# leodd/Lifted-Hybrid-Variational-Inference

Hardware: AMD Instinct MI355X
Metric: lbp_sweeps_per_sec_10M_edge_hybrid_mrf (higher is better)
Workload: dtype f64

## Files before the change

include/lhvi.h:

```cpp
#ifndef LHVI_H
#define LHVI_H

#include <stddef.h>
#include <stdint.h>

#ifdef __cplusplus
extern "C" {
#endif

#define LHVI_ABI_VERSION 30
#define LHVI_MAX_ARITY 6

#define LHVI_OK 0
#define LHVI_E_ARG (-1)
#define LHVI_E_LAUNCH (-2)
#define LHVI_E_UNSUPPORTED (-3)
#define LHVI_E_NODEVICE (-4)
#define LHVI_E_NOT_PD (-5)

#define LHVI_POT_GENERIC 0
#define LHVI_POT_TABLE 1
#define LHVI_POT_GAUSSIAN 2
#define LHVI_POT_QUADRATIC 3
#define LHVI_POT_HYBRID_QUADRATIC 4
#define LHVI_POT_LINEAR_GAUSSIAN 5
#define LHVI_POT_X2 6
#define LHVI_POT_XY 7
#define LHVI_POT_MLN 8
#define LHVI_POT_MLN_HARD 9
#define LHVI_POT_IMAGE_NODE 10
#define LHVI_POT_IMAGE_EDGE 11

typedef struct lhvi_graph {
    int32_t V, F, E, nnz;
    const int32_t* fac_ptr;
    const int32_t* edge_var;
    const int32_t* edge_fac;
    const int32_t* edge_canon;
    const int32_t* var_ptr;
    const int32_t* var_edge;
    const double* edge_count;
    const int32_t* fac_pot;
    const double* var_value;
    const int32_t* var_dom;
    const double* var_mult;
    const double* fac_mult;
    int32_t D;
    const int32_t* dom_cont;
    const double* dom_lo;
    const double* dom_hi;
    const int32_t* dom_ptr;
    const double* dom_val;
    const double* edge_value;
    const int32_t* slot_var;
    const int32_t* hub_vars;
    int32_t n_hubs;
} lhvi_graph_t;
#define LHVI_HUB_DEGREE 64

typedef struct lhvi_pots {
    int32_t P;
    const int32_t* kind;
    const int32_t* off;
// ... 8 lines not shown


int lhvi_gabp_init(const lhvi_graph_t* g, double* f2v, double* v2f, void* stream);
int lhvi_gabp_v2f(const lhvi_graph_t* g, const double* f2v, double* v2f, void* stream);
int lhvi_gabp_f2v(const lhvi_graph_t* g, const lhvi_pots_t* pots, const double* v2f, double* f2v, void* stream);
int lhvi_gabp_run(const lhvi_graph_t* g, const lhvi_pots_t* pots, double* f2v, double* v2f, int iterations, void* stream);
typedef struct lhvi_gabp_plan {
    const int32_t* pslot;
    const int32_t* info;
    const double* count;
    int32_t n_hub_rows;
    const int32_t* rec;
    const double* pot_words;
    const int32_t* seg;
    int32_t n_seg;
} lhvi_gabp_plan_t;
size_t lhvi_gabp_pull_workspace_bytes(const lhvi_graph_t* g);
int lhvi_gabp_pull(const lhvi_graph_t* g, const lhvi_pots_t* pots, const lhvi_gabp_plan_t* plan, const double* v_prev,
                   double* v_next, int first, void* stream);
int lhvi_gabp_run_pull(const lhvi_graph_t* g, const lhvi_pots_t* pots, const lhvi_gabp_plan_t* plan, double* f2v, double* v2f,
                       int iterations, void* ws, size_t ws_bytes, void* stream);

int lhvi_gabp_graph_create(const lhvi_graph_t* g, const lhvi_pots_t* pots, const lhvi_gabp_plan_t* plan, double* f2v, double* v2f,
                           double* mu_var, int iterations, void* ws, size_t ws_bytes, void** handle_out);
int lhvi_gabp_graph_launch(void* handle, void* stream);
int lhvi_gabp_graph_destroy(void* handle);

int lhvi_gabp_marginals(const lhvi_graph_t* g, const double* f2v, double* mu_var, void* stream);

size_t lhvi_log_likelihood_workspace_bytes(const lhvi_graph_t* g);
int lhvi_log_likelihood(const lhvi_graph_t* g, const lhvi_pots_t* pots, const double* x, double* out, void* ws, size_t ws_bytes,
                        void* stream);


#define LHVI_PBP_EP 1u
#define LHVI_PBP_EPBP_DISCRETE 2u
#define LHVI_PBP_SKIP_TERMS 16u
#define LHVI_PBP_LEAVE_ROOM 256u
#define LHVI_PBP_CQ 512u
#define LHVI_PBP_BOUNDARY_TOTALS 2048u
#define LHVI_PBP_NO_UNIQ 4096u
#define LHVI_PBP_V2F_RECORDS 8192u
#define LHVI_PBP_WIDE_PAIRS 16384u
#define LHVI_PBP_SHARE_CUS 32768u
#define LHVI_PBP_NO_GRID 128u
#define LHVI_PBP_FUSED_RECORDS16 131072u
#define LHVI_PBP_F2V_HEAVY 262144u
#define LHVI_PBP_F2V_SMALL 524288u
#define LHVI_PBP_F2V_PAIR 1048576u
#define LHVI_PBP_F2V_FAST 2097152u
#define LHVI_PBP_F2V_CQ 4194304u
#define LHVI_PBP_F2V_GENERIC 8388608u
#define LHVI_PBP_F2V_ALL (LHVI_PBP_F2V_HEAVY | LHVI_PBP_F2V_SMALL | LHVI_PBP_F2V_PAIR | LHVI_PBP_F2V_FAST | LHVI_PBP_F2V_CQ | LHVI_PBP_F2V_GENERIC)
#define LHVI_PBP_POW2_GROUPS 65536u

typedef struct lhvi_pbp {
    int32_t n;
    int32_t T;
    uint32_t flags;
    double var_threshold;
    double max_log_value;
    const double* particles;
    const double* old_particles;
    const int32_t* np;
    const uint8_t* uniq;
    const double* q;
    const int32_t* fast_edges;
    int32_t n_fast;
    const int32_t* generic_edges;
    int32_t n_generic;
    int32_t generic_pts_log2;
    const void* fast_desc;
    const void* heavy_desc;
    int32_t n_heavy;
    const void* light_desc;
    int32_t n_light;
    const int32_t* bslot;
    const int32_t* brow_ptr;
    const int64_t* brow_off;
    const int32_t* brow_peer;
    const double* recv;
    int32_t rank;
    const double* var_degree;
    int32_t var_lo, var_hi;
    uint32_t* f2v_ticket;
    const int32_t* prop_desc;
    int32_t n_prop_desc;
    const void* pair_desc;
    int32_t n_pair;
    const void* cq_desc;
    int32_t n_cq;
    const int32_t* v2f_wide;
    int32_t n_v2f_wide;
    const int32_t* v2f_narrow;
    int32_t n_v2f_narrow;
    const int32_t* v2f_hub;
    int32_t n_v2f_hub;
    const int32_t* v2f_mid16;
    int32_t n_v2f_mid16;
    const int32_t* v2f_mid32;
    int32_t n_v2f_mid32;
    const int32_t* prop_hub;
    int32_t n_prop_hub;
    double* prop_partial;
    const int32_t* resample_vars;
    int32_t n_resample_vars;
// ... 400 lines not shown
```

lifted-hybrid-variational-inference_amd/csrc/pbp.hip:

```cpp
#include "common.hpp"
#include "potential.hpp"
#include "fastmath.hpp"
#include "cq.hpp"
#include "gk21.hpp"

namespace lhvi {

__device__ __forceinline__ double wave_sum(double v) { return dpp_wave_reduce(v, SumOp()); }
__device__ __forceinline__ double wave_max(double v) { return dpp_wave_reduce(v, MaxOp()); }
__device__ __forceinline__ int wave_sum_i(int v) {
#pragma unroll
    for (int off = 32; off > 0; off >>= 1) v += __shfl_xor(v, off);
    return v;
}

constexpr double PAD_LOG_TERM = -6.0e5;

__host__ __device__ __forceinline__ int var_first(const lhvi_pbp_t& s) { return s.var_hi > s.var_lo ? s.var_lo : 0; }
__host__ __device__ __forceinline__ int var_limit(const lhvi_graph_t& g, const lhvi_pbp_t& s) { return s.var_hi > s.var_lo ? s.var_hi : g.V; }

__device__ __forceinline__ double norm_pdf_std(double x, double mu, double sig) {
    const double u = (x - mu) / sig;
    return exp(-u * u * 0.5) / (2.506628274631 * sig);
}
// ... 2697 lines not shown
#pragma unroll
        for (int off = PW; off < 64; off <<= 1) { fs += __shfl_xor(fs, off); fm += __shfl_xor(fm, off); }
    } else if (PW == 16 && SL == 1) { fs = (ps[0] + ps[1]) + (ps[2] + ps[3]); fm = (pm[0] + pm[1]) + (pm[2] + pm[3]); }
    else if (PW == 16) {
        const double s01 = (sub == 0 ? ps[0] : ps[1]), s23 = (sub == 0 ? ps[2] : ps[3]);
        const double m01 = (sub == 0 ? pm[0] : pm[1]), m23 = (sub == 0 ? pm[2] : pm[3]);
        fs = (s01 + __shfl_xor(s01, 16)) + (s23 + __shfl_xor(s23, 16));
        fm = (m01 + __shfl_xor(m01, 16)) + (m23 + __shfl_xor(m23, 16));
    } else { fs = ps[0] + ps[1]; fm = pm[0] + pm[1]; }
    fs = 1.0 / fs;
    const double mu_new = fs * fm, var_new = fs;
    if (on && j == 0) { q[2 * v] = mu_new; q[2 * v + 1] = var_new; }
    if constexpr (LATE_TABLE) {
        static_assert(LOG_TAB_N <= BLOCK, "one table entry per thread");
        if (threadIdx.x < LOG_TAB_N) { sh_log[threadIdx.x].inv_c = tab_inv; sh_log[threadIdx.x].log_c = tab_log; }
        __syncthreads();
    }
    const double mu_b = __shfl(mu_new, first_lane), sd_b = sqrt_pos(__shfl(var_new, first_lane));
    double x = 0.0;
    if (valid) {
        double zc, zs;
        philox_normal_pair(seed, gid ? (uint64_t)gid[v] : (uint64_t)v, (uint32_t)(W == 64 ? j & 31 : j), iteration, sh_log, zc, zs);
        if (W == 64 && (j & 32)) zc = zs;
        x = fmin(fmax(fma(sd_b, zc, mu_b), dlo), dhi) + 0.0;
        out[(int64_t)v * n + j] = x;
    }
    int u = valid;
    if constexpr (W == 64) {
        volatile uint8_t* owner = sh_owner + ((threadIdx.x >> 6) << FUSED64_HASH_BITS);
        const int xlo = __double2loint(x), xhi = __double2hiint(x);
        const uint32_t h = (((uint32_t)xlo * 0x9E3779B1u) ^ ((uint32_t)xhi * 0x85EBCA6Bu)) >> (32 - FUSED64_HASH_BITS);
        if (valid) owner[h] = (uint8_t)lane;
        LHVI_WAVE_SYNC();
        const bool suspect = valid && owner[h] != (uint8_t)lane;
        const uint64_t live = __ballot(valid);
        uint64_t todo = __ballot(suspect), dp = 0;
        while (todo) {
            const int k = __builtin_ctzll(todo);
            const int klo = __builtin_amdgcn_readlane(xlo, k), khi = __builtin_amdgcn_readlane(xhi, k);
            const uint64_t same = __ballot(xlo == klo && xhi == khi) & live;
            dp |= same & (same - 1);
            todo &= ~same;
        }
        u = valid && !((dp >> lane) & 1);
    } else {
        for (int k = 0; k + 1 < W; ++k) {
            const double xk = __shfl(x, first_lane + k);
            if (k < j && k < np && xk == x) u = 0;
        }
    }
    if (on && j < n) uniq[(int64_t)v * n + j] = (uint8_t)u;
}

}

#include "gmkl_dev.hpp"

namespace lhvi {

struct BeliefQ {
    const lhvi_graph_t& g; const lhvi_pots_t& pots; const lhvi_pbp_t& s; const double* __restrict__ v2f; const QueryRows& rows;
    int64_t i; int v; double logz; bool valid;

    template <class C> __device__ __forceinline__ void scan(const C&, const gmkl::Row&, gmkl::Scan& sc) const {
        sc.anyq = true;
        sc.bad = sc.bad || !valid;
    }
    __device__ __forceinline__ static int slots(const gmkl::Row&) { return 0; }
    template <class C> __device__ __forceinline__ void load_resident(const C&, const gmkl::Row&) const {}
    template <class C> __device__ __forceinline__ void eval(const C&, const gmkl::Row&, double x, double& m, double& sum) const {
        m = query_log_belief(g, pots, s, v2f, rows, i, v, x) - logz, sum = 1.0;
    }
};

__global__ void __launch_bounds__(WAVE, 2) pbp_kl_kernel(lhvi_graph_t g, lhvi_pots_t pots, lhvi_pbp_t s, const double* __restrict__ v2f,
                                                      QueryRows rows, const int32_t* __restrict__ row_var,
                                                      const double* __restrict__ logz, int32_t Kp, const double* __restrict__ wp,
                                                      const double* __restrict__ mup, const double* __restrict__ varp,
                                                      const double* __restrict__ a, const double* __restrict__ b, double epsabs,
                                                      double epsrel, double* __restrict__ kl, double* __restrict__ abserr,
                                                      int32_t* __restrict__ status, int32_t* __restrict__ neval) {
    __shared__ gmkl::Shared sh;
    const int64_t r = blockIdx.x;
    if (threadIdx.x == 0) {
        sh.in = gmkl::Row{Kp, 0, wp + r * Kp, mup + r * Kp, varp + r * Kp, nullptr, nullptr, nullptr, a[r], b[r], epsabs, epsrel};
        sh.kl = kl + r, sh.abserr = abserr ? abserr + r : nullptr;
        sh.status = status ? status + r : nullptr, sh.neval = neval ? neval + r : nullptr;
    }
    __syncthreads();
    gmkl::Row in = sh.in;
    in.Kp = Kp, in.Kq = 0;
    const int v = row_var[r];
    const double lz = logz[r];
    bool valid = v >= 0 && v < g.V && fabs(lz) <= DBL_MAX;
    if (valid) valid = is_hidden(g.var_value[v]) && g.dom_cont[g.var_dom[v]] != 0;
    const BeliefQ q{g, pots, s, v2f, rows, r, v, lz, valid};
    gmkl::DevCtx<BeliefQ> ctx(sh, (int)threadIdx.x, q);
    gmkl::kl_row(in, ctx, sh.kl, sh.abserr, sh.status, sh.neval);
}

static int validate_pbp(const lhvi_graph_t* g, const lhvi_pbp_t* s) {
    if (!g || !s) return LHVI_E_ARG;
    if (g->V < 0 || g->E < 0 || s->n <= 0 || s->T < 0) return LHVI_E_ARG;
    if (g->V > 0 && (!g->var_ptr || !g->var_edge || !g->var_value || !g->var_dom || !g->dom_cont || !g->dom_ptr ||
                     !s->particles || !s->np)) return LHVI_E_ARG;
    if (s->var_hi > s->var_lo ? (s->var_lo < 0 || s->var_hi > g->V) : (s->var_lo != 0 || s->var_hi != 0)) return LHVI_E_ARG;
// ... 384 lines not shown
                       row_var, xtol / 3.0, maxfun, xout, fout, nfev);
    return check_launch();
}

int lhvi_pbp_var_fused(const lhvi_graph_t* g, const lhvi_pbp_t* s, const double* f2v, double* v2f, double* eta, double* q,
                       const int64_t* var_gid, uint64_t seed, uint32_t iteration, double* particles_out, uint8_t* uniq_out,
                       const int32_t* desc, int32_t n16, int32_t n32_t32, int32_t n32_t64, void* stream) {
    if (int rc = validate_pbp(g, s)) return rc;
    if (!f2v || !v2f || !eta || !q || !particles_out || !uniq_out || !s->uniq || !s->q || !g->dom_lo || !g->dom_hi || !g->dom_val) return LHVI_E_ARG;
    if (n16 < 0 || n32_t32 < 0 || n32_t64 < 0 || s->n > 32 || s->bslot || s->var_hi > s->var_lo || particles_out == s->particles) return LHVI_E_ARG;
    if ((int64_t)n16 + n32_t32 + n32_t64 == 0) return LHVI_OK;
    if (!desc) return LHVI_E_ARG;
    hipStream_t st = as_stream(stream);
    const bool ep = (s->flags & LHVI_PBP_EP) != 0;
#define LHVI_FUSED(W, PW, list, cnt)                                                                                                  \
    if ((cnt) > 0) {                                                                                                                  \
        const dim3 grid(grid_for(((int64_t)(cnt) + WAVE / (W) - 1) / (WAVE / (W)) * WAVE));                                          \
        if (ep && r16) hipLaunchKernelGGL((pbp_var_fused_kernel<W, PW, true, true>), grid, dim3(BLOCK), 0, st, *g, *s, f2v, v2f, eta, q, var_gid, \
                                   seed, iteration, particles_out, uniq_out, list, cnt);                                             \
        else if (ep) hipLaunchKernelGGL((pbp_var_fused_kernel<W, PW, true, false>), grid, dim3(BLOCK), 0, st, *g, *s, f2v, v2f, eta, q, var_gid, \
                                   seed, iteration, particles_out, uniq_out, list, cnt);                                             \
        else if (r16) hipLaunchKernelGGL((pbp_var_fused_kernel<W, PW, false, true>), grid, dim3(BLOCK), 0, st, *g, *s, f2v, v2f, eta, q, var_gid,   \
                                seed, iteration, particles_out, uniq_out, list, cnt);                                                \
        else hipLaunchKernelGGL((pbp_var_fused_kernel<W, PW, false, false>), grid, dim3(BLOCK), 0, st, *g, *s, f2v, v2f, eta, q, var_gid,   \
                                seed, iteration, particles_out, uniq_out, list, cnt);                                                \
    }
    const bool r16 = (s->flags & LHVI_PBP_FUSED_RECORDS16) != 0;
    const int64_t rw = r16 ? 16 : 8;
    LHVI_FUSED(16, 16, desc, n16)
    LHVI_FUSED(32, 16, desc + rw * (int64_t)n16, n32_t32)
    LHVI_FUSED(32, 32, desc + rw * ((int64_t)n16 + n32_t32), n32_t64)
#undef LHVI_FUSED
    return check_launch();
}

int lhvi_pbp_var_fused64(const lhvi_graph_t* g, const lhvi_pbp_t* s, const double* f2v, double* v2f, double* eta, double* q,
                         const int64_t* var_gid, uint64_t seed, uint32_t iteration, double* particles_out, uint8_t* uniq_out,
                         const int32_t* desc, int32_t n64_t32, int32_t n64_t64, void* stream) {
    if (int rc = validate_pbp(g, s)) return rc;
    if (!f2v || !v2f || !eta || !q || !particles_out || !uniq_out || !s->uniq || !s->q || !g->dom_lo || !g->dom_hi || !g->dom_val) return LHVI_E_ARG;
    if (n64_t32 < 0 || n64_t64 < 0 || s->n <= 32 || s->n > 64 || s->bslot || s->var_hi > s->var_lo || particles_out == s->particles) return LHVI_E_ARG;
    if ((int64_t)n64_t32 + n64_t64 == 0) return LHVI_OK;
    if (!desc) return LHVI_E_ARG;
    hipStream_t st = as_stream(stream);
    const bool ep = (s->flags & LHVI_PBP_EP) != 0;
#define LHVI_FUSED64(PW, list, cnt)                                                                                                   \
    if ((cnt) > 0) {                                                                                                                  \
        const dim3 grid(grid_for((int64_t)(cnt) * WAVE));                                                                             \
        if (ep) hipLaunchKernelGGL((pbp_var_fused_kernel<64, PW, true, true>), grid, dim3(BLOCK), 0, st, *g, *s, f2v, v2f, eta, q, var_gid, \
                                   seed, iteration, particles_out, uniq_out, list, cnt);                                             \
        else hipLaunchKernelGGL((pbp_var_fused_kernel<64, PW, false, true>), grid, dim3(BLOCK), 0, st, *g, *s, f2v, v2f, eta, q, var_gid,   \
                                seed, iteration, particles_out, uniq_out, list, cnt);                                                \
    }
    LHVI_FUSED64(16, desc, n64_t32)
    LHVI_FUSED64(32, desc + 16 * (int64_t)n64_t32, n64_t64)
#undef LHVI_FUSED64
    return check_launch();
}

int lhvi_pbp_quad(const lhvi_graph_t* g, const lhvi_pots_t* pots, const lhvi_pbp_t* s, const double* v2f, int64_t nq,
                  const int32_t* row_var, const int64_t* qptr, const int32_t* qedge, const double* qmult, const double* lo,
                  const double* hi, double epsabs, double epsrel, double* z, double* abserr, int32_t* status, void* stream) {
    if (int rc = validate_pbp(g, s)) return rc;
    if (!pots || !v2f || nq < 0 || !(epsabs >= 0.0) || !(epsrel >= 0.0)) return LHVI_E_ARG;
    if (nq == 0) return LHVI_OK;
    if (!row_var || !lo || !hi || !z) return LHVI_E_ARG;
    if (qptr && (!qedge || !qmult)) return LHVI_E_ARG;
    QueryRows rows{row_var, qptr, qedge, qmult};
    hipLaunchKernelGGL(pbp_quad_kernel, dim3(grid_for(nq)), dim3(BLOCK), 0, as_stream(stream), *g, *pots, *s, v2f, nq, rows, row_var,
                       lo, hi, epsabs, epsrel, z, abserr, status);
    return check_launch();
}

int lhvi_pbp_kl(const lhvi_graph_t* g, const lhvi_pots_t* pots, const lhvi_pbp_t* s, const double* v2f, int64_t nq,
                const int32_t* row_var, const int64_t* qptr, const int32_t* qedge, const double* qmult, const double* logz,
                int32_t Kp, const double* wp, const double* mup, const double* varp, const double* a, const double* b,
                double epsabs, double epsrel, double* kl, double* abserr, int32_t* status, int32_t* neval, void* stream) {
    if (int rc = validate_pbp(g, s)) return rc;
    if (!pots || !v2f || nq < 1 || nq > 0x7fffffff || Kp < 1 || !(epsabs >= 0.0) || !(epsrel >= 0.0)) return LHVI_E_ARG;
    if (!row_var || !logz || !wp || !mup || !varp || !a || !b || !kl) return LHVI_E_ARG;
    if (g->V < 1 || !g->dom_lo || !g->dom_hi || !g->dom_val) return LHVI_E_ARG;
    if (qptr && (!qedge || !qmult)) return LHVI_E_ARG;
    QueryRows rows{row_var, qptr, qedge, qmult};
    hipLaunchKernelGGL(pbp_kl_kernel, dim3((unsigned)nq), dim3(WAVE), 0, as_stream(stream), *g, *pots, *s, v2f, rows, row_var, logz,
                       Kp, wp, mup, varp, a, b, epsabs, epsrel, kl, abserr, status, neval);
    return check_launch();
}

}
```

lifted-hybrid-variational-inference_amd/lhvi/_abi.py:

```python
from __future__ import annotations

import ctypes as C
import os

import numpy as np

_HERE = os.path.dirname(os.path.abspath(__file__))
LIB_PATH = os.environ.get('LHVI_LIB') or os.path.join(os.path.dirname(_HERE), 'csrc', 'liblhvi.so')

c_i32p = C.c_void_p
c_f64p = C.c_void_p


class LhviError(RuntimeError):
    pass


class GraphStruct(C.Structure):
    _fields_ = [
        ('V', C.c_int32), ('F', C.c_int32), ('E', C.c_int32), ('nnz', C.c_int32),
        ('fac_ptr', C.c_void_p), ('edge_var', C.c_void_p), ('edge_fac', C.c_void_p), ('edge_canon', C.c_void_p),
        ('var_ptr', C.c_void_p), ('var_edge', C.c_void_p), ('edge_count', C.c_void_p), ('fac_pot', C.c_void_p),
        ('var_value', C.c_void_p), ('var_dom', C.c_void_p), ('var_mult', C.c_void_p), ('fac_mult', C.c_void_p),
        ('D', C.c_int32),
# ... 15 lines not shown
    _fields_ = [
        ('n', C.c_int32), ('T', C.c_int32), ('flags', C.c_uint32),
        ('var_threshold', C.c_double), ('max_log_value', C.c_double),
        ('particles', C.c_void_p), ('old_particles', C.c_void_p), ('np', C.c_void_p), ('uniq', C.c_void_p),
        ('q', C.c_void_p),
        ('fast_edges', C.c_void_p), ('n_fast', C.c_int32), ('generic_edges', C.c_void_p), ('n_generic', C.c_int32),
        ('generic_pts_log2', C.c_int32), ('fast_desc', C.c_void_p), ('heavy_desc', C.c_void_p), ('n_heavy', C.c_int32), ('light_desc', C.c_void_p), ('n_light', C.c_int32),
        ('bslot', C.c_void_p), ('brow_ptr', C.c_void_p), ('brow_off', C.c_void_p), ('brow_peer', C.c_void_p),
        ('recv', C.c_void_p), ('rank', C.c_int32), ('var_degree', C.c_void_p),
        ('var_lo', C.c_int32), ('var_hi', C.c_int32),
        ('f2v_ticket', C.c_void_p),
        ('prop_desc', C.c_void_p), ('n_prop_desc', C.c_int32),
        ('pair_desc', C.c_void_p), ('n_pair', C.c_int32),
        ('cq_desc', C.c_void_p), ('n_cq', C.c_int32),
        ('v2f_wide', C.c_void_p), ('n_v2f_wide', C.c_int32), ('v2f_narrow', C.c_void_p), ('n_v2f_narrow', C.c_int32),
        ('v2f_hub', C.c_void_p), ('n_v2f_hub', C.c_int32),
        ('v2f_mid16', C.c_void_p), ('n_v2f_mid16', C.c_int32), ('v2f_mid32', C.c_void_p), ('n_v2f_mid32', C.c_int32),
        ('prop_hub', C.c_void_p), ('n_prop_hub', C.c_int32), ('prop_partial', C.c_void_p),
        ('resample_vars', C.c_void_p), ('n_resample_vars', C.c_int32),
        ('small16_desc', C.c_void_p), ('n_small16', C.c_int32), ('small32_desc', C.c_void_p), ('n_small32', C.c_int32),
        ('halo_off', C.c_void_p), ('halo_buf', C.c_void_p),
    ]


class ViStruct(C.Structure):
    _fields_ = [
        ('K', C.c_int32), ('T', C.c_int32), ('Dmax', C.c_int32), ('quirks', C.c_int32),
        ('gh_x', C.c_void_p), ('gh_w', C.c_void_p), ('w', C.c_void_p), ('eta_c', C.c_void_p), ('eta_d', C.c_void_p),
        ('obs_var', C.c_void_p), ('var_N', C.c_void_p),
        ('fac_list', C.c_void_p), ('n_cc', C.c_int32), ('n_grp3', C.c_int32), ('n_grp6', C.c_int32), ('n_rest3', C.c_int32),
        ('n_rest6', C.c_int32), ('n_tiny', C.c_int32), ('tiny_par_words', C.c_int32), ('edge_axis', C.c_void_p),
    ]


class ViOptStruct(C.Structure):
    _fields_ = [(n, C.c_void_p) for n in ('w_tau', 'w', 'eta_c', 'tau_d', 'eta_d', 'm_w', 's_w', 'm_c', 's_c', 'm_d', 's_d',
                                          'g_w', 'g_c', 'g_d', 'fe')] + \
               [(n, C.c_double) for n in ('lr', 'b1', 'b2', 'eps', 'var_min')] + [('t', C.c_int32)]


PBP_EP = 1
PBP_EPBP_DISCRETE = 2
PBP_SKIP_TERMS = 16
PBP_NO_GRID = 128
PBP_LEAVE_ROOM = 256
PBP_BOUNDARY_TOTALS = 2048
PBP_CQ = 512
PBP_NO_UNIQ = 4096
PBP_V2F_RECORDS = 8192
PBP_WIDE_PAIRS = 16384
PBP_SHARE_CUS = 32768
PBP_POW2_GROUPS = 65536
PBP_FUSED_RECORDS16 = 131072
PBP_F2V_HEAVY = 262144
PBP_F2V_SMALL = 524288
PBP_F2V_PAIR = 1048576
PBP_F2V_FAST = 2097152
PBP_F2V_CQ = 4194304
PBP_F2V_GENERIC = 8388608
PBP_F2V_ALL = PBP_F2V_HEAVY | PBP_F2V_SMALL | PBP_F2V_PAIR | PBP_F2V_FAST | PBP_F2V_CQ | PBP_F2V_GENERIC
ABI_VERSION = 30
PBP_DESC_BYTES = 128
COLOR_HASH, COLOR_SORT = 0, 1
HUB_DEGREE = 64
VI_GROUP_SLOTS, VI_GROUP_COMP, VI_TINY_NODES, VI_TINY_K, VI_TINY_PAR = 24, 48, 32, 2, 3072

class MwsStruct(C.Structure):
    _fields_ = [('T', C.c_int32), ('max_flips', C.c_int32), ('epsilon', C.c_double), ('noise_std', C.c_double),
                ('seed', C.c_uint64), ('try_id', C.c_void_p), ('disc', C.c_void_p), ('n_disc', C.c_int32),
                ('num', C.c_void_p), ('n_num', C.c_int32), ('fac_class', C.c_void_p), ('x', C.c_void_p), ('best_x', C.c_void_p),
                ('cur_score', C.c_void_p), ('best_score', C.c_void_p), ('status', C.c_void_p), ('err_flip', C.c_void_p),
                ('rec_score', C.c_void_p), ('rec_zero', C.c_void_p), ('rec_ticks', C.c_void_p)] + \
               [(n, C.c_void_p) for n in ('rp_init', 'rp_clause', 'rp_walk', 'rp_walk_k', 'rp_noise', 'rp_post', 'out_score',
                                          'out_unsat', 'out_winner', 'out_accept', 'out_val')]


class ExactStruct(C.Structure):
    _fields_ = [('Nd', C.c_int32), ('Nc', C.c_int32), ('M', C.c_int64), ('dstates', C.c_void_p), ('dstride', C.c_void_p),
                ('n_quad', C.c_int32), ('quad_ptr', C.c_void_p), ('quad_desc', C.c_void_p), ('quad_par', C.c_void_p),
                ('n_tab', C.c_int32), ('tab_ptr', C.c_void_p), ('tab_desc', C.c_void_p), ('tab_par', C.c_void_p)]


class GibbsStruct(C.Structure):
    _fields_ = [('ex', ExactStruct), ('dstate_off', C.c_void_p), ('vt_ptr', C.c_void_p), ('vt_fac', C.c_void_p),
                ('vh_ptr', C.c_void_p), ('vh_fac', C.c_void_p), ('n_hyb', C.c_int32), ('hyb_quad', C.c_void_p),
                ('hyb_off', C.c_void_p), ('table_doubles', C.c_int32), ('max_states', C.c_int32), ('table_scratch', C.c_void_p),
                ('disc_block_its', C.c_int32), ('num_burnin', C.c_int32), ('num_samples', C.c_int32), ('seed', C.c_uint64)]


E_NOT_PD = -5
EXACT_MAX_NC = 64
GAUSS_EXACT_NB = 64
GAUSS_CHAIN_MAX_BLOCK = 128

MIX_MAX_K, MIX_TILE, MIX_ROWS = 128, 64, 4
MIX_GAUSSIAN, MIX_VI = 0, 1
GMFIT_MAX_K = 16
GMKL_MAX_PANELS = 1024
GMKL_LOGQ = C.CFUNCTYPE(C.c_double, C.c_double, C.c_int64, C.c_void_p)
VI_GAUSSIAN_PDF = 2
NPVI_MAX_K, NPVI_MAX_SLOTS = 16, 24


class NpviOptStruct(C.Structure):
    _fields_ = [(n, C.c_void_p) for n in ('tau', 'theta_c', 'rho', 'm_tau', 's_tau', 'm_c', 's_c', 'm_rho', 's_rho', 'g_tau', 'g_c',
                                          'g_rho', 'obj', 'w', 'eta_c', 'eta_d', 'mu_lo', 'mu_hi')] + \
               [('lvar_lo', C.c_double), ('lvar_hi', C.c_double), ('var_count', C.c_void_p), ('fac_count', C.c_void_p)] + \
               [(n, C.c_double) for n in ('lr', 'b1', 'b2', 'eps')] + [('t', C.c_int32), ('max_slots', C.c_int32), ('max_arity', C.c_int32)]


class MixStruct(C.Structure):
    _fields_ = [('V', C.c_int32), ('K', C.c_int32), ('Dmax', C.c_int32), ('nstates', C.c_void_p), ('logw', C.c_void_p),
                ('rec', C.c_void_p), ('lpi', C.c_void_p), ('pi', C.c_void_p)]

# ... 336 lines not shown
```

lifted-hybrid-variational-inference_amd/lhvi/pbp.py:

```python
from __future__ import annotations

import os
from math import e, log, sqrt

import numpy as np

from . import _abi, pbp_plan, pbp_query
from .flat import flatten

_F2V_LONG = _abi.PBP_F2V_HEAVY | _abi.PBP_F2V_SMALL
_F2V_SHORT = _abi.PBP_F2V_PAIR | _abi.PBP_F2V_FAST | _abi.PBP_F2V_CQ | _abi.PBP_F2V_GENERIC
F2V_SCHEDULES = {
    'one': (('main', _abi.PBP_F2V_ALL, 0, False),),
    'timed': (('main', _F2V_LONG, 0, True), ('main', _F2V_SHORT, 0, False)),
    'overlap': (('side', _F2V_SHORT, 0, False), ('main', _F2V_LONG, _abi.PBP_SHARE_CUS, True)),
}


def _stream(st):
    return _abi.stream_ptr() if st is None else st


class _ParticleSweep:
    var_threshold = 3
    max_log_value = 700
    _epbp_discrete = True
    verbose = False
    listed_proposal = True
    dynamic_f2v = True
    paired_light = True
    cq_routing = True
    small_f2v = True
    long_grid_min_edges = 1 << 16
    listed_resample = True
    sliced_proposal = True
    prop_slice = 64
    packed_v2f = True
    overlap_f2v = True
    overlap_min_heavy = 1 << 16
    fused_var_kernel = True
    fused_max_particles = 64
    exact_queries = False
    map_mode = 'fminbound'
    var_gid = None
    _side = None
    _query_f2v = None
    _stable_partition = False
    _ground = None

    def _setup(self, graph_like, flat=None, edge_key=None, sides='vf', edge_skip=None, owned=None):
        flat = flat if flat is not None else flatten(graph_like, require_device_potentials=True)
        self.flat = flat
        self.dg = dg = _abi.DeviceGraph(flat)
        torch = _abi.require_gpu()
        n = self.n
        plan = pbp_plan.var_side_plan(flat, n, owned=owned, opts=self._plan_options())
        self.np_host, self.T = plan.np_host, plan.T
        S = n + self.T
        self.f2v = dg.zeros(flat.E, S)
        self.v2f = dg.zeros(flat.E, n)
        self.eta = dg.zeros(flat.E, 2)
        self.q_dev = dg.zeros(flat.V, 2)
        self.particles = dg.zeros(flat.V, n)
        self.old_particles = dg.zeros(flat.V, n)
        self.uniq = torch.zeros(flat.V, n, dtype=torch.uint8, device=dg.device)
        self.f2v_ticket = torch.zeros(16, dtype=torch.int32, device=dg.device)
        self.flags = (_abi.PBP_EP if self.proposal_approximation == 'EP' else 0) | \
                     (_abi.PBP_EPBP_DISCRETE if self._epbp_discrete else 0) | \
                     (_abi.PBP_CQ if self.cq_routing and bool((flat.pot_kind == 8).any()) else 0) | \
                     (_abi.PBP_POW2_GROUPS if os.environ.get('LHVI_PBP_POW2_GROUPS', '0') == '1' else 0) | \
                     plan.flags
        self._views, self._batched = {}, {}
        self._draws = 0
        self._static_rows = False
        self.var_lists = plan.on(_abi.upload(plan.host), dg.zeros(plan.n_prop_partial, 2) if plan.n_prop_partial else None)
        for name, value in self.var_lists.named().items():
            setattr(self, name, value)
        self._has_f_side = 'f' in sides
        self.f2v_lists = pbp_plan.F2vLists.empty(torch.zeros(1, dtype=torch.int32, device=dg.device))
        if self._has_f_side:
            cls = torch.zeros(max(flat.E, 1), dtype=torch.uint8, device=dg.device)
            _abi.check(_abi.lib().lhvi_pbp_classify(dg.g, dg.p, self._struct(), _abi.ptr(cls), _abi.stream_ptr()))
            self.f2v_lists = pbp_plan.f_side_plan(
                cls[:flat.E], flat, self.np_host, describe=self._describe,
                describe_cq=lambda edges: self._describe(edges, 'lhvi_pbp_describe_cq', 2 * _abi.PBP_DESC_BYTES),
                skip=None if edge_skip is None else _abi.to_dev(np.ascontiguousarray(edge_skip, dtype=bool)),
                key=None if edge_key is None else _abi.to_dev(np.ascontiguousarray(edge_key, dtype=np.int32)),
                paired_light=self.paired_light, small_f2v=self.small_f2v, long_grid_min_edges=self.long_grid_min_edges)
        for name, value in self.f2v_lists.named().items():
            setattr(self, name, value)

    def _describe(self, edges, entry='lhvi_pbp_describe', nbytes=_abi.PBP_DESC_BYTES):
        torch = _abi.require_gpu()
        k = int(edges.numel())
        desc = torch.empty(k * nbytes, dtype=torch.uint8, device=edges.device)
        _abi.check(getattr(_abi.lib(), entry)(self.dg.g, self.dg.p, self._struct(), _abi.ptr(edges), k, _abi.ptr(desc), _abi.stream_ptr()))
        return desc

    def _plan_options(self):
        env = os.environ.get
        return pbp_plan.PlanOptions(
            sampler_on_device=self.sampler == 'device', listed_proposal=self.listed_proposal, listed_resample=self.listed_resample,
            sliced_proposal=self.sliced_proposal, prop_slice=self.prop_slice, packed_v2f=self.packed_v2f,
            v2f_records=env('LHVI_PBP_V2F_REC', '1') != '0',
            fused=self.fused_var_kernel and env('LHVI_PBP_FUSED', '1') != '0',
            fused_max_particles=int(env('LHVI_PBP_FUSED_MAX', self.fused_max_particles)),
            fused_records16=env('LHVI_PBP_FUSED_REC16', '1') != '0')

    def _struct(self, var_range=None, leave_room=False):
        s = _abi.PbpStruct()
        s.n, s.T, s.flags = self.n, self.T, self.flags | (_abi.PBP_LEAVE_ROOM if leave_room else 0)
        s.var_threshold, s.max_log_value = float(self.var_threshold), float(self.max_log_value)
        s.particles, s.old_particles = _abi.ptr(self.particles), _abi.ptr(self.old_particles)
        s.uniq, s.q = _abi.ptr(self.uniq), _abi.ptr(self.q_dev)
        self.f2v_lists.install(s)
        if var_range is None:
            self.var_lists.install(s, self.listed_proposal)
        else:
            self.var_lists.install_range(s, *var_range)
        s.f2v_ticket = _abi.ptr(self.f2v_ticket) if self.dynamic_f2v else None
        return s

    def _launch_init(self, s, st=None):
# ... 948 lines not shown
```

Before: 70.20.

## Add paired-variable fused64 kernel processing two variables per wave

```diff
diff --git a/include/lhvi.h b/include/lhvi.h
--- a/include/lhvi.h
+++ b/include/lhvi.h
@@ -8,7 +8,7 @@
 extern "C" {
 #endif
 
-#define LHVI_ABI_VERSION 30
+#define LHVI_ABI_VERSION 31
 #define LHVI_MAX_ARITY 6
 
 #define LHVI_OK 0
@@ -123,6 +123,7 @@
 #define LHVI_PBP_F2V_CQ 4194304u
 #define LHVI_PBP_F2V_GENERIC 8388608u
 #define LHVI_PBP_F2V_ALL (LHVI_PBP_F2V_HEAVY | LHVI_PBP_F2V_SMALL | LHVI_PBP_F2V_PAIR | LHVI_PBP_F2V_FAST | LHVI_PBP_F2V_CQ | LHVI_PBP_F2V_GENERIC)
+#define LHVI_PBP_FUSED64_SINGLE 1024u
 #define LHVI_PBP_POW2_GROUPS 65536u
 
 typedef struct lhvi_pbp {
diff --git a/lifted-hybrid-variational-inference_amd/csrc/pbp.hip b/lifted-hybrid-variational-inference_amd/csrc/pbp.hip
--- a/lifted-hybrid-variational-inference_amd/csrc/pbp.hip
+++ b/lifted-hybrid-variational-inference_amd/csrc/pbp.hip
@@ -2773,6 +2773,329 @@
     if (on && j < n) uniq[(int64_t)v * n + j] = (uint8_t)u;
 }
 
+#ifndef LHVI_FUSED64_PAIR_WAVES
+#define LHVI_FUSED64_PAIR_WAVES 6
+#endif
+#ifndef LHVI_FUSED64_PAIR_EARLY
+#define LHVI_FUSED64_PAIR_EARLY 1
+#endif
+#ifndef LHVI_FUSED64_PAIR_DRAW
+#define LHVI_FUSED64_PAIR_DRAW 1
+#endif
+struct Fused64Args {
+    int32_t n, S, count;
+    uint32_t iteration;
+    double var_threshold, max_log_value;
+    uint64_t seed;
+    const double* particles;
+    const uint8_t* uniq;
+    const double* q_in;
+    const double* edge_count;
+    const int32_t* var_edge;
+    const double* dom_val;
+    const double* f2v;
+    double* v2f;
+    double* eta;
+    double* q;
+    const int64_t* gid;
+    double* out;
+    uint8_t* uniq_out;
+    const int32_t* list;
+};
+struct Fused64Var {
+    int v, deg, gb, T, np, lo;
+    double dlo, dhi, q0, q1;
+    uint64_t gid;
+    int e[FUSED_CH64];
+};
+struct Fused64Loads {
+    double x, mm[FUSED_CH64], b0, b1, g0, g1, xg0, xg1;
+    int pre_e;
+    bool uq;
+};
+
+template <bool LIFTED>
+__global__ void __launch_bounds__(BLOCK) __attribute__((amdgpu_waves_per_eu(LHVI_FUSED64_PAIR_WAVES, 8)))
+pbp_var_fused64_pair_kernel(Fused64Args a) {
+    static_assert(FUSED_CH64 == 4, "a chunk is the four lane groups of a proposal pass");
+    constexpr int CH = FUSED_CH64, PW = 16;
+    __shared__ LogRec sh_log[LOG_TAB_N];
+    __shared__ uint8_t sh_owner[(BLOCK / WAVE) << FUSED64_HASH_BITS];
+    static_assert(LOG_TAB_N <= BLOCK, "one table entry per thread");
+    double tab_inv = 0.0, tab_log = 0.0;
+    if (threadIdx.x < LOG_TAB_N) { tab_inv = LOG_TAB[2 * threadIdx.x]; tab_log = LOG_TAB[2 * threadIdx.x + 1]; }
+    const auto store_table = [&] { if (threadIdx.x < LOG_TAB_N) { sh_log[threadIdx.x].inv_c = tab_inv; sh_log[threadIdx.x].log_c = tab_log; } };
+    const int lane = threadIdx.x & 63;
+    const int wave = __builtin_amdgcn_readfirstlane(threadIdx.x >> 6);
+    const int64_t item = (int64_t)blockIdx.x * (BLOCK / WAVE) + wave;
+#define LHVI_FUSED64_ARG(field) heavy_arg_reload<decltype(Fused64Args::field)>(offsetof(Fused64Args, field))
+    const int n = a.n, S = a.S;
+    constexpr bool lifted = LIFTED;
+    const bool onA = 2 * item < a.count, onB = 2 * item + 1 < a.count;
+    const int sub = lane / PW, tl = lane % PW;
+
+    if (!onA) {
+        store_table();
+        __syncthreads();
+        return;
+    }
+    auto fetch = [&](int64_t k, bool on) {
+        Fused64Var r;
+        const int4* r4 = reinterpret_cast<const int4*>(a.list + 16 * k);
+        const int4 ra = r4[0], rb = r4[1], rc = r4[2], rd = r4[3];
+        r.v = ra.x; r.deg = on ? ra.y : 0; r.gb = ra.z; r.T = on ? ra.w : 0;
+        r.dlo = __hiloint2double(rb.y, rb.x); r.dhi = __hiloint2double(rb.w, rb.z);
+        r.np = on ? rc.x : 0; r.lo = rc.y;
+        r.e[0] = 0 < r.deg ? rc.z : 0; r.e[1] = 1 < r.deg ? rc.w : 0; r.e[2] = 2 < r.deg ? rd.x : 0; r.e[3] = 3 < r.deg ? rd.y : 0;
+        r.q0 = a.q_in[2 * r.v]; r.q1 = a.q_in[2 * r.v + 1];
+        r.gid = a.gid ? (uint64_t)a.gid[r.v] : (uint64_t)r.v;
+        return r;
+    };
+    auto pick = [&](const int* ee) { return sub == 0 ? ee[0] : sub == 1 ? ee[1] : sub == 2 ? ee[2] : ee[3]; };
+    auto chunk_edges = [&](const Fused64Var& r, int c, int* ee) {
+        const int32_t* var_edge = LHVI_FUSED64_ARG(var_edge);
+#pragma unroll
+        for (int i = 0; i < CH; ++i) ee[i] = c * CH + i < r.deg ? __builtin_amdgcn_readfirstlane(var_edge[r.lo + c * CH + i]) : 0;
+    };
+    auto edge_count = [&](int e) { return LHVI_FUSED64_ARG(edge_count)[e]; };
+    auto chunk_rows = [&](const Fused64Var& r, const int* ee, double* mm) {
+        const uint32_t off = lane < r.np ? (uint32_t)lane : 0u;
+#pragma unroll
+        for (int i = 0; i < CH; ++i) mm[i] = row_load(scalar_row(a.f2v + (int64_t)ee[i] * S), off);
+    };
+    auto issue_rows = [&](const Fused64Var& r, Fused64Loads& l) {
+        const bool valid = lane < r.np;
+        l.x = 0.0; l.uq = false;
+        if (valid) {
+            l.x = a.particles[(int64_t)r.v * n + lane];
+            l.uq = a.uniq[(int64_t)r.v * n + lane] != 0;
+        }
+        chunk_rows(r, r.e, l.mm);
+    };
+    auto issue_pass = [&](const Fused64Var& r, Fused64Loads& l) {
+        const int t0 = min(tl, max(r.T - 1, 0)), t1 = min(tl + PW, max(r.T - 1, 0));
+        l.pre_e = pick(r.e);
+        const double* msg = a.f2v + (int64_t)l.pre_e * S + n;
+        l.b0 = a.eta[2 * l.pre_e]; l.b1 = a.eta[2 * l.pre_e + 1];
+        l.g0 = msg[t0]; l.g1 = msg[t1];
+        const double* dom_val = LHVI_FUSED64_ARG(dom_val);
+        l.xg0 = dom_val[r.gb + t0]; l.xg1 = dom_val[r.gb + t1];
+    };
+    auto step1 = [&](const Fused64Var& r, const Fused64Loads& l, auto multi) {
+        constexpr bool MULTI = decltype(multi)::value;
+        const int deg = r.deg;
+        const bool valid = lane < r.np;
+        const int nch = MULTI ? (deg + CH - 1) / CH : 1;
+        const bool uq = l.uq;
+        {
+            double logw = 0.0;
+            if (valid) {
+                const double LOG_1E200 = 460.51701859880916;
+                const double sd = sqrt_pos(r.q1);
+                const double rsd = rcp_newton(sd), log_norm = log_pos(2.506628274631 * sd);
+                if (l.x == r.dlo || l.x == r.dhi) logw = -LOG_1E200;
+                else {
+                    const double u = (l.x - r.q0) * rsd;
+                    logw = fmin(u * u * 0.5 + log_norm, LOG_1E200);
+                }
+            }
+            double total = 0.0;
+#pragma unroll
+            for (int i = 0; i < CH; ++i) {
+                const double m = valid ? l.mm[i] : 0.0;
+                if (i < deg) {
+#pragma clang fp contract(off)
+                    total += lifted ? m * edge_count(r.e[i]) : m;
+                }
+            }
+            for (int c = 1; c < nch; ++c) {
+                int ee[CH];
+                double mm[CH];
+                chunk_edges(r, c, ee);
+                chunk_rows(r, ee, mm);
+#pragma unroll
+                for (int i = 0; i < CH; ++i) {
+                    const double m = valid ? mm[i] : 0.0;
+                    if (c * CH + i < deg) {
+#pragma clang fp contract(off)
+                        total += lifted ? m * edge_count(ee[i]) : m;
+                    }
+                }
+            }
+            const double rcnt = rcp_newton(fmax((double)__builtin_popcountll(__ballot(uq)), 1.0));
+            auto emit = [&](int c, const int* ee, const double* mm) {
+#pragma unroll
+                for (int i = 0; i < CH; ++i) {
+                    const int k = c * CH + i;
+                    if (k >= deg) break;
+                    const double m = valid ? mm[i] : 0.0;
+                    const double res = (total - m) + logw;
+                    const double mean = wave_sum(uq ? res : 0.0) * rcnt;
+                    double shift = mean;
+                    if (__ballot(uq && (res - mean > a.max_log_value))) {
+                        const double mx = wave_max(uq ? res : -__builtin_huge_val());
+                        if (mx - mean > a.max_log_value) shift = mx - a.max_log_value;
+                    }
+                    if (valid) row_store(scalar_row(a.v2f + (int64_t)ee[i] * n), (uint32_t)lane, res - shift);
+                }
+            };
+            emit(0, r.e, l.mm);
+            for (int c = 1; c < nch; ++c) {
+                int ee[CH];
+                double mm[CH];
+                chunk_edges(r, c, ee);
+                chunk_rows(r, ee, mm);
+                emit(c, ee, mm);
+            }
+        }
+    };
+    auto step2 = [&](const Fused64Var& r, const Fused64Loads& l, bool on, double& mu_new, double& var_new, auto multi) {
+        constexpr bool MULTI = decltype(multi)::value;
+        const int deg = r.deg, T = r.T;
+        const int nch = MULTI ? (deg + CH - 1) / CH : (deg > 0 ? 1 : 0);
+        double total = 0.0;
+        if (lifted) {
+            const int32_t* var_edge = LHVI_FUSED64_ARG(var_edge);
+            for (int k = 0; k < deg; ++k) total += edge_count(var_edge[r.lo + k]);
+        } else total = (double)deg;
+        const double min_sig = total * LHVI_FUSED64_ARG(var_threshold);
+        const int t0 = min(tl, max(T - 1, 0)), t1 = min(tl + PW, max(T - 1, 0));
+        const double xg0 = l.xg0, xg1 = l.xg1;
+        double ps = 0.0, pm = 0.0;
+        for (int c = 0; c < nch; ++c) {
+            int e = l.pre_e;
+            double b0 = l.b0, b1 = l.b1, g0 = l.g0, g1 = l.g1;
+            if (MULTI && c > 0) {
+                int ee[CH];
+                chunk_edges(r, c, ee);
+                e = pick(ee);
+                const double* msg = a.f2v + (int64_t)e * S + n;
+                b0 = a.eta[2 * e]; b1 = a.eta[2 * e + 1];
+                g0 = msg[t0]; g1 = msg[t1];
+            }
+            const int k = c * CH + sub;
+            const bool live = k < deg;
+            const double e0 = b0, e1 = b1;
+            double z = 0.0, sa = 0.0, sb = 0.0;
+            if (tl < T) {
+                double w = exp(g0);
+                z += w; sa += w * xg0; sb += w * (xg0 * xg0);
+            }
+            __builtin_amdgcn_sched_barrier(0);
+            if (tl + PW < T) {
+                double w = exp(g1);
+                z += w; sa += w * xg1; sb += w * (xg1 * xg1);
+            }
+            __builtin_amdgcn_sched_barrier(0);
+            z = dpp_row_reduce(z, SumOp()); sa = dpp_row_reduce(sa, SumOp()); sb = dpp_row_reduce(sb, SumOp());
+            const double rz = rcp_newton(z);
+            double mu = sa * rz;
+            double sig = sb * rz - mu * mu;
+            if (0.0 < sig && sig < __builtin_huge_val()) {
+                sig = fmax(sig, min_sig);
+                if (live && tl == 0) { a.eta[2 * e] = mu; a.eta[2 * e + 1] = sig; }
+            } else {
+                mu = e0; sig = e1;
+            }
+            if (live) {
+#pragma clang fp contract(off)
+                const double p = rcp_newton(sig);
+                const double pmu = p * mu;
+                if (lifted) { const double cnt = edge_count(e); ps += p * cnt; pm += pmu * cnt; }
+                else { ps += p; pm += pmu; }
+            }
+        }
+        double fs = ps, fm = pm;
+#pragma unroll
+        for (int off = PW; off < 64; off <<= 1) { fs += __shfl_xor(fs, off); fm += __shfl_xor(fm, off); }
+        fs = 1.0 / fs;
+        mu_new = fs * fm; var_new = fs;
+        if (on && lane == 0) { double* q = LHVI_FUSED64_ARG(q); q[2 * r.v] = mu_new; q[2 * r.v + 1] = var_new; }
+        mu_new = readlane_f64(mu_new, 0); var_new = readlane_f64(var_new, 0);
+    };
+
+    const Fused64Var A = fetch(2 * item, true), B = fetch(onB ? 2 * item + 1 : 2 * item, onB);
+    double muA, varA, muB, varB;
+    if (A.deg <= CH && B.deg <= CH) {
+        constexpr std::false_type one_chunk{};
+        Fused64Loads la, lb;
+        issue_rows(A, la);
+        issue_pass(A, la);
+        if (LHVI_FUSED64_PAIR_EARLY) issue_rows(B, lb);
+        store_table();
+        step1(A, la, one_chunk);
+        if (LHVI_FUSED64_PAIR_EARLY) issue_pass(B, lb);
+        step2(A, la, true, muA, varA, one_chunk);
+        if (!LHVI_FUSED64_PAIR_EARLY) { issue_rows(B, lb); issue_pass(B, lb); }
+        step1(B, lb, one_chunk);
+        step2(B, lb, onB, muB, varB, one_chunk);
+    } else {
+        constexpr std::true_type chunks{};
+        store_table();
+        {
+            Fused64Loads l;
+            issue_rows(A, l);
+            issue_pass(A, l);
+            step1(A, l, chunks);
+            step2(A, l, true, muA, varA, chunks);
+        }
+        {
+            Fused64Loads l;
+            issue_rows(B, l);
+            issue_pass(B, l);
+            step1(B, l, chunks);
+            step2(B, l, onB, muB, varB, chunks);
+        }
+    }
+    __syncthreads();
+    double rowA, rowB;
+    if (!LHVI_FUSED64_PAIR_DRAW) {
+        double zc, zs;
+        philox_normal_pair(LHVI_FUSED64_ARG(seed), A.gid, (uint32_t)(lane & 31), LHVI_FUSED64_ARG(iteration), sh_log, zc, zs);
+        rowA = (lane & 32) ? zs : zc;
+        philox_normal_pair(LHVI_FUSED64_ARG(seed), B.gid, (uint32_t)(lane & 31), LHVI_FUSED64_ARG(iteration), sh_log, zc, zs);
+        rowB = (lane & 32) ? zs : zc;
+    } else {
+        const uint64_t mine = (lane >> 5) ? B.gid : A.gid;
+        double zc, zs;
+        philox_normal_pair(LHVI_FUSED64_ARG(seed), mine, (uint32_t)(lane & 31), LHVI_FUSED64_ARG(iteration), sh_log, zc, zs);
+        auto plo = __builtin_amdgcn_permlane32_swap(__double2loint(zc), __double2loint(zs), false, false);
+        auto phi = __builtin_amdgcn_permlane32_swap(__double2hiint(zc), __double2hiint(zs), false, false);
+        rowA = __hiloint2double(phi[0], plo[0]);
+        rowB = __hiloint2double(phi[1], plo[1]);
+    }
+    volatile uint8_t* owner = sh_owner + ((threadIdx.x >> 6) << FUSED64_HASH_BITS);
+    auto finish = [&](const Fused64Var& r, double z, double mu_b, double var_b) {
+        const bool valid = lane < r.np;
+        const double sd_b = sqrt_pos(var_b);
+        double x = 0.0;
+        if (valid) {
+            x = fmin(fmax(fma(sd_b, z, mu_b), r.dlo), r.dhi) + 0.0;
+            LHVI_FUSED64_ARG(out)[(int64_t)r.v * n + lane] = x;
+        }
+        const int xlo = __double2loint(x), xhi = __double2hiint(x);
+        const uint32_t h = (((uint32_t)xlo * 0x9E3779B1u) ^ ((uint32_t)xhi * 0x85EBCA6Bu)) >> (32 - FUSED64_HASH_BITS);
+        if (valid) owner[h] = (uint8_t)lane;
+        LHVI_WAVE_SYNC();
+        const bool suspect = valid && owner[h] != (uint8_t)lane;
+        const uint64_t live = __ballot(valid);
+        uint64_t todo = __ballot(suspect), dp = 0;
+        while (todo) {
+            const int k = __builtin_ctzll(todo);
+            const int klo = __builtin_amdgcn_readlane(xlo, k), khi = __builtin_amdgcn_readlane(xhi, k);
+            const uint64_t same = __ballot(xlo == klo && xhi == khi) & live;
+            dp |= same & (same - 1);
+            todo &= ~same;
+        }
+        const int u = valid && !((dp >> lane) & 1);
+        if (lane < n) LHVI_FUSED64_ARG(uniq_out)[(int64_t)r.v * n + lane] = (uint8_t)u;
+        LHVI_WAVE_SYNC();
+    };
+    finish(A, rowA, muA, varA);
+    if (onB) finish(B, rowB, muB, varB);
+#undef LHVI_FUSED64_ARG
+}
+
 }
 
 #include "gmkl_dev.hpp"
@@ -3263,7 +3586,20 @@
         else hipLaunchKernelGGL((pbp_var_fused_kernel<64, PW, false, true>), grid, dim3(BLOCK), 0, st, *g, *s, f2v, v2f, eta, q, var_gid,   \
                                 seed, iteration, particles_out, uniq_out, list, cnt);                                                \
     }
-    LHVI_FUSED64(16, desc, n64_t32)
+    if (!ep && n64_t32 > 0 && !(s->flags & LHVI_PBP_FUSED64_SINGLE)) {
+        if (!g->var_edge) return LHVI_E_ARG;
+        Fused64Args a{};
+        a.n = s->n; a.S = s->n + s->T; a.count = n64_t32; a.iteration = iteration;
+        a.var_threshold = s->var_threshold; a.max_log_value = s->max_log_value; a.seed = seed;
+        a.particles = s->particles; a.uniq = s->uniq; a.q_in = s->q;
+        a.edge_count = g->edge_count; a.var_edge = g->var_edge; a.dom_val = g->dom_val;
+        a.f2v = f2v; a.v2f = v2f; a.eta = eta; a.q = q; a.gid = var_gid; a.out = particles_out; a.uniq_out = uniq_out; a.list = desc;
+        const dim3 grid(grid_for(((int64_t)n64_t32 + 1) / 2 * WAVE));
+        if (g->edge_count) hipLaunchKernelGGL(pbp_var_fused64_pair_kernel<true>, grid, dim3(BLOCK), 0, st, a);
+        else hipLaunchKernelGGL(pbp_var_fused64_pair_kernel<false>, grid, dim3(BLOCK), 0, st, a);
+    } else {
+        LHVI_FUSED64(16, desc, n64_t32)
+    }
     LHVI_FUSED64(32, desc + 16 * (int64_t)n64_t32, n64_t64)
 #undef LHVI_FUSED64
     return check_launch();
diff --git a/lifted-hybrid-variational-inference_amd/lhvi/_abi.py b/lifted-hybrid-variational-inference_amd/lhvi/_abi.py
--- a/lifted-hybrid-variational-inference_amd/lhvi/_abi.py
+++ b/lifted-hybrid-variational-inference_amd/lhvi/_abi.py
@@ -91,6 +91,7 @@
 PBP_SHARE_CUS = 32768
 PBP_POW2_GROUPS = 65536
 PBP_FUSED_RECORDS16 = 131072
+PBP_FUSED64_SINGLE = 1024
 PBP_F2V_HEAVY = 262144
 PBP_F2V_SMALL = 524288
 PBP_F2V_PAIR = 1048576
@@ -98,7 +99,7 @@
 PBP_F2V_CQ = 4194304
 PBP_F2V_GENERIC = 8388608
 PBP_F2V_ALL = PBP_F2V_HEAVY | PBP_F2V_SMALL | PBP_F2V_PAIR | PBP_F2V_FAST | PBP_F2V_CQ | PBP_F2V_GENERIC
-ABI_VERSION = 30
+ABI_VERSION = 31
 PBP_DESC_BYTES = 128
 COLOR_HASH, COLOR_SORT = 0, 1
 HUB_DEGREE = 64
diff --git a/lifted-hybrid-variational-inference_amd/lhvi/pbp.py b/lifted-hybrid-variational-inference_amd/lhvi/pbp.py
--- a/lifted-hybrid-variational-inference_amd/lhvi/pbp.py
+++ b/lifted-hybrid-variational-inference_amd/lhvi/pbp.py
@@ -40,6 +40,7 @@
     overlap_min_heavy = 1 << 16
     fused_var_kernel = True
     fused_max_particles = 64
+    fused64_pairs = True
     exact_queries = False
     map_mode = 'fminbound'
     var_gid = None
@@ -69,6 +70,7 @@
                      (_abi.PBP_EPBP_DISCRETE if self._epbp_discrete else 0) | \
                      (_abi.PBP_CQ if self.cq_routing and bool((flat.pot_kind == 8).any()) else 0) | \
                      (_abi.PBP_POW2_GROUPS if os.environ.get('LHVI_PBP_POW2_GROUPS', '0') == '1' else 0) | \
+                     (0 if self.fused64_pairs and os.environ.get('LHVI_PBP_FUSED64_PAIRS', '1') != '0' else _abi.PBP_FUSED64_SINGLE) | \
                      plan.flags
         self._views, self._batched = {}, {}
         self._draws = 0
```

Measured after the change: 70.46 (median of 6 runs). About the same (+0.4%).
